# cvg/nice-slam

Hardware: AMD Instinct MI355X
Metric: rendered rays/sec (fwd+bwd) per mapping iter (higher is better)
Workload: dtype f32 (f64 sample placement / depth)

## Files before the change

nice_slam_amd/csrc/nsr_bwd2.h:

```cpp
#pragma once

namespace nsr {

constexpr int kDySlots = 10;
constexpr int kDxMaxWaves = 12;
constexpr int kDxTx = 0, kDxTab = kTile * kTxS, kDxP = kDxTab + 256, kDxDP = kDxP + 48, kDxStg = kDxDP + 48;
static_assert(kDxStg % 4 == 0, "staging regions must stay 16-byte aligned");
constexpr int kDbPart = 288;
NSR_KERNEL void comp_bwd_kernel(const RenderParams P) {
    const int lane = tid() & 63, wave = tid() >> 6, nw = nthreads() >> 6;
    const long long ray = (long long)bid_x() * nw + wave;
    if (ray >= P.n_rays) return;
    const int S = P.S;
    if (!ray_live(P, ray)) {
        if (lane < S) st4(P.draw + (ray * S + lane) * 4, F4{0.f, 0.f, 0.f, 0.f});
        return;
    }
    const bool act = lane < S;
    const long long gp = ray * S + (act ? lane : 0);
    const F4 rw = act ? ld4(P.raw + gp * 4) : F4{0.f, 0.f, 0.f, 0.f};
    const double sc = P.g_scale ? P.g_scale[0] : 1.0;
    const double gD = P.d_depth ? P.d_depth[ray] * sc : 0.0, gV = P.d_var ? P.d_var[ray] * sc : 0.0, dep = P.g_depth[ray];
    float gr = 0.f, gg = 0.f, gb = 0.f;
    if (P.d_rgb) { gr = P.d_rgb[ray * 3 + 0] * (float)sc; gg = P.d_rgb[ray * 3 + 1] * (float)sc; gb = P.d_rgb[ray * 3 + 2] * (float)sc; }
    const double z = act ? P.zvals[gp] : 0.0;
    const Comp cw = comp_weights(rw.w, act, lane);
    const double dz = z - dep;
    float docc = comp_docc(cw, rw, z, dz, gD, gV, gr, gg, gb, act, lane);
    const Pos p = sample_pos(P, ray, z);
    if (!in_bound(P, p.x, p.y, p.z)) docc = 0.f;
    if (act) {
        st4(P.draw + gp * 4, F4{cw.w * gr, cw.w * gg, cw.w * gb, docc});
        store_pos(P, gp, p, z);
    }
}

template <int NTK>
NSR_DEV void gemv_t(f32x4 (&dx)[NTK], const Act<2> &dy, const float *wt, int lane) {
#pragma unroll
    for (int To = 0; To < 2; ++To) {
        f32x4 a[NTK];
#pragma unroll
        for (int Tk = 0; Tk < NTK; ++Tk) a[Tk] = to_v(ld4(wt + ((Tk * 2 + To) * 64 + lane) * 4));
#pragma unroll
        for (int r = 0; r < 4; ++r)
#pragma unroll
            for (int Tk = 0; Tk < NTK; ++Tk) dx[Tk] = mfma16(a[Tk][r], dy.t[To][r], dx[Tk]);
    }
    sched_fence();
}

struct DxIn {
    F4 dr;
    unsigned m0, m1;
};
NSR_DEV DxIn dx_load(const RenderParams &P, const float *acts_pass, long long tile, int pt, int g) {
    DxIn I;
    const long long gp = tile * kTile + pt;
    const long long q = gp < P.n_points_total ? gp : 0;
    I.dr = ld4(P.draw + q * 4);
    const float *mp = acts_pass + ((q >> 4) * kActSlots + kActMask) * 256 + ((q & 15) * 4 + g) * 4;
    I.m0 = __builtin_bit_cast(unsigned, mp[0]);
    I.m1 = __builtin_bit_cast(unsigned, mp[1]);
    return I;
}
NSR_DEV void dx_keep(const DxIn &I) {
    keep_alive(I.dr.w); keep_alive(__builtin_bit_cast(float, I.m1));
}

template <int KIND, bool PARAMS, bool RAYS>
NSR_DEV void dx_pass(const RenderParams &P, int bi, int nbp, int gb) {
    constexpr bool XYZ = KIND != NSR_COARSE;
    constexpr int NOUT = nout_of(KIND);
    char *lds = lds_base();
    const int lane = tid() & 63, wave = uniform(tid() >> 6), nw = nthreads() >> 6;
    const int pt = lane & 15, g = lane >> 4;
    float *aux = reinterpret_cast<float *>(lds);
    float *wt = aux + AUX_FLOATS;
    float *stg = wt + packedT_total(KIND);
    float *Sw = stg + wave * kDxStg;
    const int tail_off = uniform((int)(stg + nw * kDxStg - reinterpret_cast<float *>(lds)));
    const int gl_off = (KIND == NSR_COARSE && P.lds_grid_floats > 0) ? tail_off : -1;
    float *gl = gl_off >= 0 ? reinterpret_cast<float *>(lds) + gl_off : nullptr;
    const bool use_hot = KIND != NSR_COARSE && P.hot_z[KIND] > 0.f && P.grid[KIND].dfeat != nullptr;
    const HotTab hot{use_hot ? tail_off : -1, P.hot_slots};
    int *tcnt = reinterpret_cast<int *>(stg + nw * kDxStg + (KIND == NSR_COARSE ? P.lds_grid_floats : P.hot_slots * kHotRow));
    const GridDev &G = P.grid[KIND];
    const DecDev &D = P.dec[KIND];
    const bool do_grid = G.dfeat != nullptr;
    if (!do_grid && !PARAMS && !RAYS) return;
    const Dbg dbg{P.dbg ? P.dbg + ((long long)gb * kDxMaxWaves + wave) * 64 : nullptr};
    dbg.stamp(0);
    constexpr long long sstride = 256;
    const float *acts_pass = P.acts + (long long)act_pass(KIND) * P.act_tiles * kActSlots * 256;
    const long long ntiles = (P.n_points_total + kTile - 1) / kTile;
    const long long t0 = ntiles * bi / nbp, tend = ntiles * (bi + 1) / nbp;
    long long tile = t0 + wave;
    const bool pre = tile < tend && tile_live(P, tile);
    DxIn cur;
    if (pre) cur = dx_load(P, acts_pass, tile, pt, g);
    copy_f4<AUX_FLOATS / 4>(aux, D.packed);
    copy_f4_dma<packedT_total(KIND) / 4>(wt, D.packed + AUX_FLOATS + packed_total(KIND));
    if (gl) for (int i = tid(); i < P.lds_grid_floats; i += nthreads()) gl[i] = 0.f;
    if (use_hot) hot_init(hot);
    if (tid() == 0) tcnt[0] = nw;
    dma_wait<0>();
    block_sync();
    dbg.stamp(1);
    float *dys = P.dy + (long long)act_pass(KIND) * P.act_tiles * kDySlots * 256;
    const bool need_dc = do_grid || RAYS;
    float aB[kET][3];
#pragma unroll
    for (int k = 0; k < kET; ++k) { aB[k][0] = 0.f; aB[k][1] = 0.f; aB[k][2] = 0.f; }

    auto claim = [&]() -> long long {
        for (;;) {
            int k = 0;
            if (lane == 0) k = atomic_fetch_add_lds_i(tcnt, 1);
            const long long t = t0 + shfl_i(k, 0);
            if (t >= tend || tile_live(P, t)) return t;
        }
    };
    const float dr_scale = (!P.draw_scaled && P.g_scale) ? (float)P.g_scale[0] : 1.f;
    if (!pre) {
        tile = claim();
        if (tile < tend) cur = dx_load(P, acts_pass, tile, pt, g);
    }
    if (tile < tend) dx_keep(cur);
    while (tile < tend) {
        loop_fence();
        const long long nxt = claim();
        const bool has_next = nxt < tend;
        DxIn nx = cur;
        if (has_next) nx = dx_load(P, acts_pass, nxt, pt, g);
        const long long gp = tile * kTile + pt;
        const bool active = gp < P.n_points_total;
        const double *pp = P.pd + (active ? gp : 0) * 4;
        const double cpx = pp[0], cpy = pp[1], cpz = pp[2], cz = pp[3];
        dbg.stamp(2);
        const unsigned mw0 = active ? cur.m0 : 0u, mw1 = active ? cur.m1 : 0u;
        const float dsc = active ? dr_scale : 0.f;
        float d_out[4] = {0.f, 0.f, 0.f, 0.f};
        if (NOUT == 1) d_out[0] = cur.dr.w * dsc;
        else { d_out[0] = cur.dr.x * dsc; d_out[1] = cur.dr.y * dsc; d_out[2] = cur.dr.z * dsc; }
        Act<2> dh;
#pragma unroll
        for (int T = 0; T < 2; ++T) {
            f32x4 v = f4zero();
#pragma unroll
            for (int n = 0; n < (NOUT == 1 ? 1 : 3); ++n) {
                const F4 w = ld4(aux + AUX_WO + n * 32 + 16 * T + 4 * g);
                v[0] = fmaf(w.x, d_out[n], v[0]); v[1] = fmaf(w.y, d_out[n], v[1]);
                v[2] = fmaf(w.z, d_out[n], v[2]); v[3] = fmaf(w.w, d_out[n], v[3]);
            }
            dh.t[T] = v;
        }
        Act<2> dc, dY0, dY3;
        act_zero(dc); act_zero(dY0); act_zero(dY3);
        float *dyp = dys + tile * (kDySlots * 256) + (pt * 4 + g) * 4;
#pragma unroll
        for (int I = 4; I >= 0; --I) {
            if (XYZ && need_dc) gemv_t<2>(dc.t, dh, wt + xyzT_u(I), lane);
            const Act<2> dY = apply_mask(dh, I < 4 ? mw0 : mw1, I < 4 ? 8 * I : 0);
            if (PARAMS && active) {
                st4(dyp + (2 * I) * sstride, to_F4(dY.t[0]));
                st4(dyp + (2 * I + 1) * sstride, to_F4(dY.t[1]));
            }
            if (I == 3) dY3 = dY;
            if (I == 0) dY0 = dY;
            if (!XYZ) {
                if (I == 3 && need_dc) gemv_t<2>(dc.t, dY, wt + nox_mat(NW3C).pk, lane);
                if (I == 0 && need_dc) gemv_t<2>(dc.t, dY, wt + nox_mat(NW0).pk, lane);
            }
            if (I > 0) {
                Act<2> nd;
                act_zero(nd);
                if (XYZ) gemv_t<2>(nd.t, dY, wt + xyzT_wh(I - 1), lane);
                else gemv_t<2>(nd.t, dY, wt + nox_mat(I == 1 ? NW1 : (I == 2 ? NW2 : (I == 3 ? NW3H : NW4))).pk, lane);
                dh = nd;
            }
        }
        dbg.stamp(3);
        const float px = (float)cpx, py = (float)cpy, pz = (float)cpz;
        float dpe[3] = {0.f, 0.f, 0.f};
        if (XYZ && PARAMS && ballot64(active) != 0ull) {
            if (g == 0) { Sw[kDxP + pt] = px; Sw[kDxP + 16 + pt] = py; Sw[kDxP + 32 + pt] = pz; }
            wave_fence();
            const f32x4 qx = to_v(ld4(Sw + kDxP + 4 * g)), qy = to_v(ld4(Sw + kDxP + 16 + 4 * g)), qz = to_v(ld4(Sw + kDxP + 32 + 4 * g));
            f32x4 sx = f4zero(), sy = f4zero(), sz = f4zero();
#pragma unroll
            for (int Tk = 0; Tk < kET; ++Tk) {
                f32x4 e0 = f4zero(), e3 = f4zero();
#pragma unroll
                for (int To = 0; To < 2; ++To) {
                    const f32x4 a0 = to_v(ld4(wt + xyzT_w0() + ((Tk * 2 + To) * 64 + lane) * 4));
                    const f32x4 a3 = to_v(ld4(wt + xyzT_w3e() + ((Tk * 2 + To) * 64 + lane) * 4));
#pragma unroll
                    for (int r = 0; r < 4; ++r) {
                        e0 = mfma16(dY0.t[To][r], a0[r], e0);
                        e3 = mfma16(dY3.t[To][r], a3[r], e3);
                    }
                }
                sched_fence();
                const F4 b = load_b1(aux, 16 * Tk + pt);
                const f32x4 darg = (e0 + e3) * cos_dx4(vfma(qz, splat(b.z), vfma(qy, splat(b.y), qx * splat(b.x))));
#pragma unroll
                for (int r = 0; r < 4; ++r) {
                    aB[Tk][0] = fmaf(darg[r], qx[r], aB[Tk][0]); aB[Tk][1] = fmaf(darg[r], qy[r], aB[Tk][1]);
                    aB[Tk][2] = fmaf(darg[r], qz[r], aB[Tk][2]);
                }
                if (RAYS) { sx = vfma(darg, splat(b.x), sx); sy = vfma(darg, splat(b.y), sy); sz = vfma(darg, splat(b.z), sz); }
            }
            if (RAYS) {
#pragma unroll
                for (int m = 1; m < 16; m <<= 1)
#pragma unroll
                    for (int r = 0; r < 4; ++r) { sx[r] += shfl_xor(sx[r], m); sy[r] += shfl_xor(sy[r], m); sz[r] += shfl_xor(sz[r], m); }
                if (pt == 0) { st4(Sw + kDxDP + 4 * g, to_F4(sx)); st4(Sw + kDxDP + 16 + 4 * g, to_F4(sy)); st4(Sw + kDxDP + 32 + 4 * g, to_F4(sz)); }
                wave_fence();
                dpe[0] = Sw[kDxDP + pt]; dpe[1] = Sw[kDxDP + 16 + pt]; dpe[2] = Sw[kDxDP + 32 + pt];
            }
            wave_fence();
        } else if (XYZ && RAYS) {
            f32x4 dE[kET];
#pragma unroll
            for (int Tk = 0; Tk < kET; ++Tk) dE[Tk] = f4zero();
            gemv_t<kET>(dE, dY0, wt + xyzT_w0(), lane);
            gemv_t<kET>(dE, dY3, wt + xyzT_w3e(), lane);
            float ax = 0.f, ay = 0.f, az = 0.f;
#pragma unroll
            for (int Tk = 0; Tk < kET; ++Tk) {
                const B4 b = load_b4(aux, 4 * Tk + g);
                const f32x4 darg = dE[Tk] * cos_dx4(vfma(splat(pz), b.z, vfma(splat(py), b.y, splat(px) * b.x)));
#pragma unroll
                for (int r = 0; r < 4; ++r) { ax = fmaf(darg[r], b.x[r], ax); ay = fmaf(darg[r], b.y[r], ay); az = fmaf(darg[r], b.z[r], az); }
                sched_fence();
            }
            dpe[0] = red_g(ax); dpe[1] = red_g(ay); dpe[2] = red_g(az);
        }
        dbg.stamp(4);
        Lvl L;
        if (need_dc) L = make_level(G, cpx, cpy, cpz);
        const unsigned live = (do_grid && G.gmask) ? gmask_bits(G, L, g) : 3u;
        float dux = 0.f, duy = 0.f, duz = 0.f;
        if (RAYS) coord_grad(G, L, g, dc, dux, duy, duz);
        dx_keep(nx);
        keep_alive_d(cpx); keep_alive_d(cpy); keep_alive_d(cpz); keep_alive_d(cz);
        dbg.stamp(5);
        if (do_grid)
            scatter_merged(G, L, lane, dc, active, Sw + kDxTx, Sw + kDxTab, gl_off, hot, (float)cz < P.hot_z[KIND], live);
        dbg.stamp(6);
        if (RAYS) {
            double v[6];
            const bool mine = active && g == 0;
            v[0] = mine ? (double)dux * (2.0 * G.inv[0]) + (double)dpe[0] : 0.0;
            v[1] = mine ? (double)duy * (2.0 * G.inv[1]) + (double)dpe[1] : 0.0;
            v[2] = mine ? (double)duz * (2.0 * G.inv[2]) + (double)dpe[2] : 0.0;
            v[3] = v[0] * cz; v[4] = v[1] * cz; v[5] = v[2] * cz;
            if ((P.S & (kTile - 1)) == 0) {
#pragma unroll
                for (int m = 1; m < 16; m <<= 1)
#pragma unroll
                    for (int q = 0; q < 6; ++q) v[q] += shfl_xor_d(v[q], m);
                if (lane == 0 && active) {
                    const long long ray = (long long)((unsigned)gp / (unsigned)P.S);
#pragma unroll
                    for (int q = 0; q < 3; ++q) {
                        atomic_add_global(P.d_rays_o + ray * 3 + q, (float)v[q]);
                        atomic_add_global(P.d_rays_d + ray * 3 + q, (float)v[3 + q]);
                    }
                }
            } else if (mine) {
// ... 305 lines not shown
        const int i = lane & 15, g = lane >> 4;
        if (kWe) {
            img_tile(img, xyz_mat(CD, XW0), 0, WAVE, we[0], i, g); img_tile(img, xyz_mat(CD, XW0), 1, WAVE, we[1], i, g);
            img_tile(img, xyz_mat(CD, XW3E), 0, WAVE, we[2], i, g); img_tile(img, xyz_mat(CD, XW3E), 1, WAVE, we[3], i, g);
        }
        if (kB0) {
#pragma unroll
            for (int T = 0; T < 2; ++T) { const float v = red_g4(vb0[T]); if (g == 0) img[bias_off(KIND, 0) + 16 * T + i] = v; }
        }
        if (WJ) {
            img_tile(img, xyz_mat(CD, hid_of(WJ)), ROW, 0, wh[0], i, g); img_tile(img, xyz_mat(CD, hid_of(WJ)), ROW, 1, wh[1], i, g);
            const float v = red_g4(vb);
            if (g == 0) img[bias_off(KIND, WJ) + 16 * ROW + i] = v;
        }
        if (W2J) {
            img_tile(img, xyz_mat(CD, hid_of(W2J)), ROW, 0, w2[0], i, g); img_tile(img, xyz_mat(CD, hid_of(W2J)), ROW, 1, w2[1], i, g);
            const float v = red_g4(vb2);
            if (g == 0) img[bias_off(KIND, W2J) + 16 * ROW + i] = v;
        }
        if (ROW == 0) {
#pragma unroll
            for (int Tk = 0; Tk < 2; ++Tk)
#pragma unroll
                for (int Tc = 0; Tc < NC; ++Tc) {
                    const f32x4 o = pu[Tk][Tc] + to_v(ld4(comb + (((GJ - 1) * 2 + Tk) * NC + Tc) * 256 + lane * 4));
#pragma unroll
                    for (int r = 0; r < 4; ++r) img[xyz_fcw(CD, GJ - 1) + (16 * Tk + 4 * g + r) * CD + 16 * Tc + i] = o[r];
                }
            if (i == 0) {
#pragma unroll
                for (int Tk = 0; Tk < 2; ++Tk) {
                    if (WJ) {
                        const f32x4 o = pv[Tk] + to_v(ld4(comb + kCombB + (WJ - 1) * 32 + 16 * Tk + 4 * g));
#pragma unroll
                        for (int r = 0; r < 4; ++r) img[xyz_fcb(CD, WJ - 1) + 16 * Tk + 4 * g + r] = o[r];
                    }
                    if (W2J) {
                        const f32x4 o = pv2[Tk] + to_v(ld4(comb + kCombB + (W2J - 1) * 32 + 16 * Tk + 4 * g));
#pragma unroll
                        for (int r = 0; r < 4; ++r) img[xyz_fcb(CD, W2J - 1) + 16 * Tk + 4 * g + r] = o[r];
                    }
                }
            }
        }
        if (kOut) {
            float gsum[NO][NC], bsum[NO];
#pragma unroll
            for (int n = 0; n < NO; ++n) {
#pragma unroll
                for (int T = 0; T < 2; ++T) { const float v = red_g4(wo[n][T]); if (g == 0) img[wo_off(KIND) + n * 32 + 16 * T + i] = v; }
                bsum[n] = red_g4(bo[n]);
                if (lane == 0) img[bo_off(KIND) + n] = bsum[n];
#pragma unroll
                for (int Tc = 0; Tc < NC; ++Tc) gsum[n][Tc] = red_g4(go[n][Tc]);
            }
            if (NOUT == 4 && lane < 32) img[wo_off(KIND) + 3 * 32 + lane] = 0.f;
            if (NOUT == 4 && lane == 0) img[bo_off(KIND) + 3] = 0.f;
#pragma unroll
            for (int kk = 0; kk < 8; ++kk) {
                const int k = 8 * g + kk;
                float wk[NO];
#pragma unroll
                for (int n = 0; n < NO; ++n) wk[n] = params[wo_off(KIND) + n * 32 + k];
#pragma unroll
                for (int Tc = 0; Tc < NC; ++Tc) {
                    float v = 0.f;
#pragma unroll
                    for (int n = 0; n < NO; ++n) v = fmaf(wk[n], gsum[n][Tc], v);
                    img[xyz_fcw(CD, 4) + k * CD + 16 * Tc + i] = v;
                }
                if (i == 0) {
                    float v = 0.f;
#pragma unroll
                    for (int n = 0; n < NO; ++n) v = fmaf(wk[n], bsum[n], v);
                    img[xyz_fcb(CD, 4) + k] = v;
                }
            }
        }
    }
};

template <int WAVE>
struct DwNoxWave {
    static constexpr int LJ = WAVE == NW3C ? 3 : (WAVE == NW3H ? 3 : (WAVE == NW4 ? 4 : WAVE));
    static constexpr bool kMat = WAVE < 6, kBias = kMat && WAVE != NW3H, kOut = WAVE == 6;
    f32x4 w[2][2];
    float vb[2], wo[2], bo, dscale;
    NSR_DEV void init(const RenderParams &P, int) {
        dscale = (!P.draw_scaled && P.g_scale) ? (float)P.g_scale[0] : 1.f;
#pragma unroll
        for (int a = 0; a < 2; ++a) { vb[a] = 0.f; wo[a] = 0.f; w[a][0] = f4zero(); w[a][1] = f4zero(); }
        bo = 0.f;
    }
    struct Ops { f32x4 a[2], x[2]; float dn[4]; };
    NSR_DEV void fetch(const DwSrc s, int lane, Ops &o) {
        const int g = lane >> 4;
        if (kMat) {
            o.a[0] = gop(s.dy + (2 * LJ) * 256, lane); o.a[1] = gop(s.dy + (2 * LJ + 1) * 256, lane);
#pragma unroll
            for (int Tk = 0; Tk < 2; ++Tk)
                o.x[Tk] = gop(s.act + ((WAVE == NW0 || WAVE == NW3C) ? kActC + Tk : 2 * (LJ - 1) + Tk) * 256, lane);
        }
        if (kOut) {
            o.x[0] = gop(s.act + 8 * 256, lane); o.x[1] = gop(s.act + 9 * 256, lane);
#pragma unroll
            for (int q = 0; q < 4; ++q) o.dn[q] = s.dr[(4 * q + g) * 4 + 3] * dscale;
        }
    }
    NSR_DEV void consume(Ops &o, int lane, int nvalid) {
        const int g = lane >> 4;
        if (nvalid < kTile) {
            if (kMat) { rag(o.a[0], g, nvalid); rag(o.a[1], g, nvalid); }
            if (kMat || kOut) { rag(o.x[0], g, nvalid); rag(o.x[1], g, nvalid); }
#pragma unroll
            for (int q = 0; q < 4; ++q) if (kOut && 4 * q + g >= nvalid) o.dn[q] = 0.f;
        }
        if (kMat) {
            if (kBias) { vb[0] += sum4(o.a[0]); vb[1] += sum4(o.a[1]); }
#pragma unroll
            for (int q = 0; q < 4; ++q)
#pragma unroll
                for (int To = 0; To < 2; ++To)
#pragma unroll
                    for (int Tk = 0; Tk < 2; ++Tk) w[To][Tk] = mfma16(o.a[To][q], o.x[Tk][q], w[To][Tk]);
        }
        if (kOut) {
#pragma unroll
            for (int q = 0; q < 4; ++q) { wo[0] = fmaf(o.dn[q], o.x[0][q], wo[0]); wo[1] = fmaf(o.dn[q], o.x[1][q], wo[1]); bo += o.dn[q]; }
        }
    }
    NSR_DEV void flush_products(const float *, float *, int) {}
    NSR_DEV void flush(float *img, const float *, const float *, int lane) {
        const int i = lane & 15, g = lane >> 4;
        if (kMat) {
            const Mat m = nox_mat(WAVE);
#pragma unroll
            for (int To = 0; To < 2; ++To)
#pragma unroll
                for (int Tk = 0; Tk < 2; ++Tk) img_tile(img, m, To, Tk, w[To][Tk], i, g);
            if (kBias) {
#pragma unroll
                for (int T = 0; T < 2; ++T) { const float v = red_g4(vb[T]); if (g == 0) img[nox_b(LJ) + 16 * T + i] = v; }
            }
        }
        if (kOut) {
#pragma unroll
            for (int T = 0; T < 2; ++T) { const float v = red_g4(wo[T]); if (g == 0) img[nox_wo() + 16 * T + i] = v; }
            const float vbo = red_g4(bo);
            if (lane == 0) img[nox_bo()] = vbo;
        }
    }
};

NSR_DEV unsigned long long dw_live_mask(const RenderParams &P, long long bi, long long step, int chunk, long long ntiles, int lane) {
    if (!P.skip_masked) return ~0ull;
    const long long t = bi + ((long long)chunk * 64 + lane) * step;
    bool live = false;
    if (t < ntiles) {
        const unsigned p0 = (unsigned)t * kTile, np = (unsigned)P.n_points_total, pe = p0 + kTile < np ? p0 + kTile : np;
        const unsigned r0 = ray_of_point(P, p0), r1 = ray_of_point(P, pe - 1);
        for (unsigned r = r0; r <= r1; ++r) live = live || P.keep[r] != 0;
    }
    return ballot64(live);
}

template <int KIND, class W>
NSR_DEV void dw_compute(const RenderParams &P, W &Wv, float *ring, int *ctl, float *img, int wave, int lane, int bi, int nbp) {
    typedef DwLay<KIND> Y;
    Wv.init(P, lane & 15);
    const long long ntiles = (P.n_points_total + kTile - 1) / kTile;
    const long long last = ntiles - 1, step = nbp;
    const int ragged = (int)(P.n_points_total & (kTile - 1));
    typename W::Ops ops;
    int k = 0;
    unsigned long long lm = ~0ull;
    const Dbg dbg{P.dbg ? P.dbg + kDwDbgOff + ((long long)bid_x() * kDxMaxWaves + wave) * 64 : nullptr};
    dbg.stamp(0);
    for (long long t = bi; t < ntiles; t += step, ++k) {
        loop_fence();
        dbg.stamp(1);
        if ((k & 63) == 0) lm = dw_live_mask(P, bi, step, k >> 6, ntiles, lane);
        while (flag_load(ctl + (k % kDwLoaders)) <= (k / kDwLoaders)) spin_pause();
        dbg.stamp(2);
        if ((lm >> (k & 63)) & 1ull) {
            Wv.fetch(dw_src<KIND>(ring + (k % kDwRing) * Y::kSlot), lane, ops);
#ifdef NSR_TS
            asm volatile("s_waitcnt lgkmcnt(0)" ::: "memory");
            dbg.stamp(9);
#endif
            Wv.consume(ops, lane, (t == last && ragged) ? ragged : kTile);
        }
        dbg.stamp(3);
        flag_store(ctl + kDwLoaders + wave, k + 1);
        dbg.stamp(4);
    }
    dbg.stamp(5);
    block_sync();
    dbg.stamp(6);
    Wv.flush_products(P.dec[KIND].params, ring, lane);
    block_sync();
    dbg.stamp(7);
    Wv.flush(img, P.dec[KIND].params, ring, lane);
    dbg.stamp(8);
}

template <int KIND>
NSR_DEV void dw_loader(const RenderParams &P, float *ring, int *ctl, int j, int lane, int bi, int nbp) {
    typedef DwLay<KIND> Y;
    const long long ntiles = (P.n_points_total + kTile - 1) / kTile;
    const long long step = nbp;
    int m = 0;
    unsigned long long lm = ~0ull;
    int chunk = -1;
    const Dbg dbg{P.dbg ? P.dbg + kDwDbgOff + ((long long)bid_x() * kDxMaxWaves + kDwCompute + j) * 64 : nullptr};
    dbg.stamp(0);
    for (long long t = bi + j * step; t < ntiles; t += kDwLoaders * step, ++m) {
        loop_fence();
        dbg.stamp(1);
        const int k = kDwLoaders * m + j;
        if ((k >> 6) != chunk) { chunk = k >> 6; lm = dw_live_mask(P, bi, step, chunk, ntiles, lane); }
        if (m >= 1) { dma_wait<0>(); flag_store(ctl + j, m); }
        if (k >= kDwRing) {
            for (;;) {
                int lo = flag_load(ctl + kDwLoaders);
#pragma unroll
                for (int w = 1; w < kDwCompute; ++w) { const int v = flag_load(ctl + kDwLoaders + w); lo = v < lo ? v : lo; }
                if (lo > k - kDwRing) break;
                spin_pause();
            }
        }
        dbg.stamp(2);
        if ((lm >> (k & 63)) & 1ull) {
            dw_issue<KIND>(P, t, ring + (k % kDwRing) * Y::kSlot, lane);
            dbg.stamp(3);
        }
        dbg.stamp(4);
    }
    dma_wait<0>();
    flag_store(ctl + j, m);
    dbg.stamp(5);
    block_sync();
    block_sync();
}

template <int KIND>
NSR_DEV void dw_pass(const RenderParams &P, int bi, int nbp) {
    float *ring = reinterpret_cast<float *>(lds_base());
    int *ctl = reinterpret_cast<int *>(ring + kDwRing * DwLay<KIND>::kSlot);
    const int lane = tid() & 63, wave = uniform(tid() >> 6);
    if (tid() < 16) ctl[tid()] = 0;
    block_sync();
    float *img = P.partials + (long long)bid_x() * P.partial_stride;
#define NSR_DW_CASE(WV)                                                                                         \
    case WV: {                                                                                                  \
        if constexpr (KIND == NSR_COARSE) { DwNoxWave<WV> W; dw_compute<KIND>(P, W, ring, ctl, img, WV, lane, bi, nbp); } \
        else { DwXyzWave<KIND, WV> W; dw_compute<KIND>(P, W, ring, ctl, img, WV, lane, bi, nbp); }                        \
        break;                                                                                                  \
    }
    switch (wave) {
        NSR_DW_CASE(0) NSR_DW_CASE(1) NSR_DW_CASE(2) NSR_DW_CASE(3) NSR_DW_CASE(4) NSR_DW_CASE(5) NSR_DW_CASE(6) NSR_DW_CASE(7)
        default: dw_loader<KIND>(P, ring, ctl, wave - kDwCompute, lane, bi, nbp); break;
    }
#undef NSR_DW_CASE
}

template <int STAGE>
NSR_KERNEL NSR_BOUNDS(64 * kDwWaves) void render_bwd_dw_kernel(const RenderParams P) {
    const int b = bid_x();
    if (STAGE == NSR_STAGE_COARSE) {
        dw_pass<NSR_COARSE>(P, b, nblk_x());
    } else {
        if (b < P.dw_beg[1]) dw_pass<NSR_MIDDLE>(P, b, P.dw_beg[1]);
        else if (b < P.dw_beg[2]) { if (STAGE >= NSR_STAGE_FINE) dw_pass<NSR_FINE>(P, b - P.dw_beg[1], P.dw_beg[2] - P.dw_beg[1]); }
        else { if (STAGE == NSR_STAGE_COLOR) dw_pass<NSR_COLOR>(P, b - P.dw_beg[2], P.dw_beg[3] - P.dw_beg[2]); }
    }
}

struct FinalJob {
    const float *images;
    const float *dbpart;
    float *dparams;
    int kind, nimg, ndx;
};
struct FinalParams {
    FinalJob job[3];
    int stride, overwrite;
};
NSR_DEV void final_store(const FinalParams &R, float *p, float v) { *p = R.overwrite ? v : *p + v; }
NSR_DEV float strided_sum(const float *p, long long stride, int first, int step, int n) {
    float s = 0.f;
    for (int k0 = first; k0 < n; k0 += 16 * step) {
        float v[16];
#pragma unroll
        for (int j = 0; j < 16; ++j) { const int k = k0 + j * step; v[j] = k < n ? p[(long long)k * stride] : 0.f; }
#pragma unroll
        for (int j = 0; j < 16; ++j) if (k0 + j * step < n) s += v[j];
    }
    return s;
}

NSR_KERNEL void bwd_finalize_kernel(const FinalParams R) {
    const FinalJob J = R.job[bid_y()];
    float *red = reinterpret_cast<float *>(lds_base());
    const int kind = J.kind, cd = cdim_of(kind);
    const int total = param_total(kind);
    const int t = tid(), nt = nthreads();
    const int lane = t & 63, slice = t >> 6, nslice = nt >> 6;
    const int e = bid_x() * 64 + lane;
    if (bid_x() * 64 >= total) return;
    float s = 0.f;
    if (e < total) {
        const int rb = kind != NSR_COARSE ? e - xyz_B(cd) : -1;
        if (rb >= 0 && rb < 3 * kE) {
            const int d = rb / kE, ch = rb - d * kE;
            s = strided_sum(J.dbpart + d * 96 + ch, kDbPart, slice, nslice, J.ndx);
        } else {
            s = strided_sum(J.images + e, R.stride, slice, nslice, J.nimg);
        }
    }
    red[t] = s;
    block_sync();
    if (slice == 0 && e < total) {
        for (int k = 1; k < nslice; ++k) s += red[k * 64 + lane];
        final_store(R, J.dparams + e, s);
    }
}

}
```

nice_slam_amd/csrc/nsr_fwd2.h:

```cpp
#pragma once

namespace nsr {

NSR_KERNEL void fwd_sample_kernel(const RenderParams P) {
    double *zs = reinterpret_cast<double *>(lds_base());
    const int lane = tid() & 63, wave = tid() >> 6, nw = nthreads() >> 6;
    const long long ray = (long long)bid_x() * nw + wave;
    const int S = P.S;
    double *zw = zs + wave * 64;
    if (ray >= P.n_rays) return;
    const bool act = lane < S;
    const int k = act ? lane : 0;
    const bool guided = depth_guided(P);
    double z = sample_candidate(P, ray, k, guided);
    if (P.n_surface > 0 && guided) {
        if (act) zw[lane] = z;
        wave_fence();
        const int rank = stable_rank(zw, S, k, z);
        wave_fence();
        if (act) zw[rank] = z;
        wave_fence();
        z = act ? zw[lane] : 0.0;
    }
    if (!act) return;
    const long long gq = ray * S + lane;
    P.zvals[gq] = z;
    store_pos(P, gq, sample_pos(P, ray, z), z);
}

template <int KIND, bool SAVE>
NSR_DEV void fwd_pass(const RenderParams &P, int bi, int nbp) {
    float *aux = reinterpret_cast<float *>(lds_base());
    float *wl = aux + AUX_FLOATS;
    int *cnt = reinterpret_cast<int *>(wl + packed_total(KIND));
    const int lane0 = tid() & 63, wave = tid() >> 6;
    const DecDev &D = P.dec[KIND];
    const Dbg dbg{P.dbg ? P.dbg + ((long long)bid_x() * 12 + wave) * 64 : nullptr};
    dbg.stamp(0);
    load_aux<KIND>(aux, D.packed);
    copy_f4_dma<packed_total(KIND) / 4>(wl, D.packed + AUX_FLOATS);
    if (tid() == 0) cnt[0] = 0;
    dma_wait<0>();
    block_sync();
    dbg.stamp(1);
    const long long ntiles = (P.n_points_total + kTile - 1) / kTile;
    const long long t0 = ntiles * bi / nbp, t1 = ntiles * (bi + 1) / nbp;
    for (;;) {
        int take = 0;
        if (lane0 == 0) take = atomic_fetch_add_lds_i(cnt, 1);
        const long long tile = t0 + shfl_i(take, 0);
        if (tile >= t1) break;
        if (!tile_live(P, tile)) continue;
        loop_fence();
        const int lane = opaque_i(lane0), pt = lane & 15, g = lane >> 4;
        const long long gp = tile * kTile + pt;
        const bool active = gp < P.n_points_total;
        const double *pp = P.pd + (active ? gp : 0) * 4;
        const double px = pp[0], py = pp[1], pz = pp[2];
        dbg.stamp(2);
        const long long sp = (SAVE && active) ? gp : -1;
        float *scr = P.draw + gp * 4;
        if (KIND == NSR_COARSE) {
            const Lvl L = make_level(P.grid[NSR_COARSE], px, py, pz);
            const Act<2> c = gather_feat(P.grid[NSR_COARSE], L, g);
            float o[1];
            const ActSink sk = act_sink(P, 0, sp, g);
            mlp_nox_fwd<SAVE>(wl, aux, c, lane, o, &sk);
            if (active && g == 0) scr[0] = o[0];
        } else {
            const float fx = (float)px, fy = (float)py, fz = (float)pz;
            if (KIND == NSR_MIDDLE) {
                const Lvl Lm = make_level(P.grid[NSR_MIDDLE], px, py, pz);
                const Act<2> cm = gather_feat(P.grid[NSR_MIDDLE], Lm, g);
                float om[1];
                const ActSink sk = act_sink(P, 0, sp, g);
                mlp_xyz_fwd<NSR_MIDDLE, SAVE>(wl, aux, fx, fy, fz, cm, lane, om, &sk);
                if (active && g == 0) scr[0] = om[0];
            } else if (KIND == NSR_FINE) {
                const Lvl Lf = make_level(P.grid[NSR_FINE], px, py, pz);
                const Act<2> cf = gather_feat(P.grid[NSR_FINE], Lf, g);
                const Lvl Lm = make_level(P.grid[NSR_MIDDLE], px, py, pz);
                const Act<2> cm = gather_feat(P.grid[NSR_MIDDLE], Lm, g);
                Act<4> cc;
                cc.t[0] = cf.t[0]; cc.t[1] = cf.t[1]; cc.t[2] = cm.t[0]; cc.t[3] = cm.t[1];
                float of[1];
                const ActSink sk = act_sink(P, 1, sp, g);
                mlp_xyz_fwd<NSR_FINE, SAVE>(wl, aux, fx, fy, fz, cc, lane, of, &sk);
                if (active && g == 0) scr[1] = of[0];
            } else {
                const Lvl Lc = make_level(P.grid[NSR_COLOR], px, py, pz);
                const Act<2> ccol = gather_feat(P.grid[NSR_COLOR], Lc, g);
                float oc[4];
                const ActSink sk = act_sink(P, 2, sp, g);
                mlp_xyz_fwd<NSR_COLOR, SAVE>(wl, aux, fx, fy, fz, ccol, lane, oc, &sk);
                if (active && g == 0) { float *rw = P.raw + gp * 4; rw[0] = oc[0]; rw[1] = oc[1]; rw[2] = oc[2]; }
            }
        }
        dbg.stamp(3);
    }
    dbg.stamp(9);
}

template <int STAGE, bool SAVE>
NSR_KERNEL NSR_BOUNDS(768) void render_fwd_pass_kernel(const RenderParams P) {
    const int b = bid_x();
    if (STAGE == NSR_STAGE_COARSE) {
        fwd_pass<NSR_COARSE, SAVE>(P, b, nblk_x());
    } else {
        if (b < P.pass_beg[1]) fwd_pass<NSR_MIDDLE, SAVE>(P, b, P.pass_beg[1]);
        else if (b < P.pass_beg[2]) { if (STAGE >= NSR_STAGE_FINE) fwd_pass<NSR_FINE, SAVE>(P, b - P.pass_beg[1], P.pass_beg[2] - P.pass_beg[1]); }
        else { if (STAGE == NSR_STAGE_COLOR) fwd_pass<NSR_COLOR, SAVE>(P, b - P.pass_beg[2], P.pass_beg[3] - P.pass_beg[2]); }
    }
}

template <int STAGE>
NSR_KERNEL void fwd_composite_kernel(const RenderParams P) {
    double *red = reinterpret_cast<double *>(lds_base());
    const int lane = tid() & 63, wave = tid() >> 6, nw = nthreads() >> 6;
    const long long rayq = (long long)bid_x() * nw + wave;
    const int S = P.S;
    double lterm = 0.0;
    if (rayq < P.n_rays && !ray_live(P, rayq)) {
        if (lane == 0) {
            P.depth[rayq] = 0.0; P.var[rayq] = 0.0;
            P.rgb[rayq * 3 + 0] = 0.f; P.rgb[rayq * 3 + 1] = 0.f; P.rgb[rayq * 3 + 2] = 0.f;
            if (P.loss && P.dl_depth) P.dl_depth[rayq] = 0.0;
            if (P.loss && P.dl_rgb) { P.dl_rgb[rayq * 3 + 0] = 0.f; P.dl_rgb[rayq * 3 + 1] = 0.f; P.dl_rgb[rayq * 3 + 2] = 0.f; }
        }
        if (P.loss && P.dl_depth && lane < S) st4(P.draw + (rayq * S + lane) * 4, F4{0.f, 0.f, 0.f, 0.f});
    } else if (rayq < P.n_rays) {
        const bool act = lane < S;
        const long long gq = rayq * S + (act ? lane : 0);
        const bool kp = !P.loss || !P.keep || P.keep[rayq];
        const float gd = (P.loss && P.loss_depth) ? P.loss_depth[rayq] : 0.f;
        float gtc[3] = {0.f, 0.f, 0.f};
        if (P.loss && STAGE == NSR_STAGE_COLOR && P.gt_color) { gtc[0] = P.gt_color[rayq * 3 + 0]; gtc[1] = P.gt_color[rayq * 3 + 1]; gtc[2] = P.gt_color[rayq * 3 + 2]; }
        double qx = 0.0, qy = 0.0, qz = 0.0, zq = 0.0;
        F4 rw = F4{0.f, 0.f, 0.f, 0.f};
        bool ins = true;
        if (act) {
            const double *pq = P.pd + gq * 4;
            qx = pq[0]; qy = pq[1]; qz = pq[2]; zq = pq[3];
            const float *scr = P.draw + gq * 4;
            float occ = scr[0];
            if (STAGE >= NSR_STAGE_FINE) occ = scr[1] + scr[0];
            if (STAGE == NSR_STAGE_COLOR) { const float *rc = P.raw + gq * 4; rw.x = rc[0]; rw.y = rc[1]; rw.z = rc[2]; }
            ins = in_bound(P, qx, qy, qz);
            rw.w = ins ? occ : 100.f;
            st4(P.raw + gq * 4, rw);
        }
        const Comp c = comp_weights(rw.w, act, lane);
        const RayOut o = composite(c, rw, zq);
        if (lane == 0) {
            P.depth[rayq] = o.depth;
            P.var[rayq] = o.var;
            P.rgb[rayq * 3 + 0] = o.cr; P.rgb[rayq * 3 + 1] = o.cg; P.rgb[rayq * 3 + 2] = o.cb;
        }
        if (P.loss) {
            const RayLoss L = mapping_loss_ray<STAGE>(P, kp, gd, gtc, o.depth, o.cr, o.cg, o.cb);
            lterm = L.term;
            if (lane == 0) {
                if (P.dl_depth) P.dl_depth[rayq] = L.gD;
                if (P.dl_rgb) { P.dl_rgb[rayq * 3 + 0] = L.g3[0]; P.dl_rgb[rayq * 3 + 1] = L.g3[1]; P.dl_rgb[rayq * 3 + 2] = L.g3[2]; }
            }
            if (P.dl_depth) {
                float docc = comp_docc(c, rw, zq, o.dz, L.gD, 0.0, L.g3[0], L.g3[1], L.g3[2], act, lane);
                if (!ins) docc = 0.f;
                if (act) st4(P.draw + gq * 4, F4{c.w * L.g3[0], c.w * L.g3[1], c.w * L.g3[2], docc});
            }
        }
    }
    if (P.loss) {
        if (lane == 0) red[wave] = lterm;
        block_sync();
        if (tid() == 0) {
            double s = 0.0;
            for (int w = 0; w < nw; ++w) s += red[w];
            if (s != 0.0) atomic_add_global_d(P.loss, s);
        }
    }
}

}
```

nice_slam_amd/csrc/nsr_kernels.h:

```cpp
#pragma once
#include "nsr_dev.h"
#include "nsr_layout.h"
#include "../../include/nsr.h"

namespace nsr {

template <int NT>
struct Act { f32x4 t[NT]; };

NSR_DEV f32x4 f4zero() { f32x4 v = {0.f, 0.f, 0.f, 0.f}; return v; }
NSR_DEV f32x4 to_v(F4 a) { f32x4 v = {a.x, a.y, a.z, a.w}; return v; }
NSR_DEV F4 to_F4(f32x4 v) { return F4{v[0], v[1], v[2], v[3]}; }
template <int NT> NSR_DEV void act_zero(Act<NT> &a) {
#pragma unroll
    for (int T = 0; T < NT; ++T) a.t[T] = f4zero();
}

NSR_DEV double tmax(double a, double b) { return (a > b || a != a) ? a : b; }
NSR_DEV double tmin(double a, double b) { return (a < b || a != a) ? a : b; }

struct GridDev {
    const float *feat;
    float *dfeat;
    const unsigned char *gmask;
    int Z, Y, X;
    double lo[3];
    double ext[3];
    double inv[3];
};

struct DecDev {
    const float *params;
    const float *packed;
    float *dparams;
};

struct RenderParams {
    int stage, n_samples, n_surface, S;
    long long n_rays;
    int rays_per_block, tiles_per_block;
    long long n_groups;
    const float *rays_o, *rays_d, *gt_depth, *gt_max;
    double blo[3], bhi[3];
    float t_uniform[NSR_MAX_SAMPLES];
    double t_surface[NSR_MAX_SAMPLES];
    GridDev grid[4];
    DecDev dec[4];
    double *depth, *var;
    float *rgb, *raw;
    double *zvals;
    float *acts;
    int acts_masks_only;
    long long n_points_total;
    long long act_tiles;
    const double *d_depth, *d_var, *g_depth;
    const double *g_scale;
    const float *d_rgb;
    float *d_rays_o, *d_rays_d;
    float *partials;
    int partial_stride;
    const float *loss_depth;
    const float *gt_color;
    const unsigned char *keep;
    double *loss;
    double *dl_depth;
    float *dl_rgb;
    float w_color;
    long long *dbg;
    float *dy;
    float *draw;
    double *pd;
    float *pf;
    float *dbpart;
    int dw_beg[4];
    int dx_beg[4];
    int draw_scaled;
    int skip_masked;
    int lds_grid_floats;
    float hot_z[4];
    int hot_slots;
    unsigned s_magic;
    int pass_beg[4];
    const double *points;
    long long n_points;
    float *out_points;
};

NSR_DEV bool ray_live(const RenderParams &P, long long ray) { return !P.skip_masked || uniform_load_u8(P.keep + ray) != 0u; }
NSR_DEV unsigned ray_of_point(const RenderParams &P, unsigned x) {
    return P.s_magic ? (unsigned)(((unsigned long long)x * P.s_magic) >> 32) : x;
}
NSR_DEV bool tile_live(const RenderParams &P, long long tile) {
    if (!P.skip_masked) return true;
    const unsigned p0 = (unsigned)uniform((int)tile) * kTile, np = (unsigned)P.n_points_total, pe = p0 + kTile < np ? p0 + kTile : np;
    const unsigned r0 = ray_of_point(P, p0), r1 = ray_of_point(P, pe - 1);
    bool live = false;
    for (unsigned r = r0; r <= r1; ++r) live = live || uniform_load_u8(P.keep + r) != 0u;
    return live;
}

template <int KIND>
NSR_DEV float aux_value(const float *__restrict__ flat, int idx) {
    float v = 0.f;
    if (idx < AUX_V) {
        const int i = idx >> 5, o = idx & 31;
        v = flat[bias_off(KIND, i) + o];
    } else if (idx < AUX_WO) {
        if (is_xyz(KIND)) { const int i = (idx - AUX_V) >> 5, o = idx & 31; v = flat[fcb_off(KIND, i) + o]; }
    } else if (idx < AUX_BO) {
        const int n = (idx - AUX_WO) >> 5, k = idx & 31;
        if (n < nout_of(KIND)) v = flat[wo_off(KIND) + n * 32 + k];
    } else if (idx < AUX_BM) {
        const int n = idx - AUX_BO;
        if (n < nout_of(KIND)) v = flat[bo_off(KIND) + n];
    } else if (is_xyz(KIND)) {
        const int rel = idx - AUX_BM, ch = (rel >> 4) * 4 + (rel & 3), d = (rel >> 2) & 3;
        if (ch < kE && d < 3) v = flat[B_off(KIND) + d * kE + ch];
    }
    return v;
}

template <int KIND>
NSR_KERNEL void pack_kernel(const float *__restrict__ flat, float *__restrict__ packed) {
    const int gidx = bid_x() * nthreads() + tid();
    if (gidx >= packed_buf_total(KIND)) return;
    if (gidx < AUX_FLOATS) { packed[gidx] = aux_value<KIND>(flat, gidx); return; }
    const int idx = gidx - AUX_FLOATS;
    float v = 0.f;
    if (idx < packed_total(KIND)) {
#pragma unroll
        for (int id = 0; id < nmat_of(KIND); ++id) {
            const Mat m = mat_of(KIND, id);
            const int rel = idx - m.pk;
            if (rel >= 0 && rel < m.nt * 512) {
                const int r = rel & 3, lane = (rel >> 2) & 63, Tp = (rel >> 8) & 1, T = rel >> 9;
                const int o = 16 * Tp + (lane & 15);
                const int k = 16 * T + 4 * (lane >> 4) + r;
                if (k < m.kcols) v = flat[m.off + o * m.stride + m.kbeg + k];
            }
        }
    } else {
        const int idt = idx - packed_total(KIND);
#pragma unroll
        for (int id = 0; id < nmatT_of(KIND); ++id) {
            const Mat m = matT_of(KIND, id);
            const int rel = idt - m.pk;
            if (rel >= 0 && rel < m.nt * 512) {
                const int r = rel & 3, lane = (rel >> 2) & 63, To = (rel >> 8) & 1, Tk = rel >> 9;
                const int o = 16 * To + 4 * (lane >> 4) + r;
                const int k = 16 * Tk + (lane & 15);
                if (k < m.kcols) v = flat[m.off + o * m.stride + m.kbeg + k];
            }
        }
    }
    packed[gidx] = v;
}

template <int NF4, int B = 4>
NSR_DEV void copy_f4(float *dst, const float *__restrict__ src) {
    const int nt = nthreads();
    int t = tid();
    for (; t + (B - 1) * nt < NF4; t += B * nt) {
        F4 v[B];
#pragma unroll
        for (int k = 0; k < B; ++k) v[k] = ld4(src + 4 * (t + k * nt));
#pragma unroll
        for (int k = 0; k < B; ++k) st4(dst + 4 * (t + k * nt), v[k]);
    }
    for (; t < NF4; t += nt) st4(dst + 4 * t, ld4(src + 4 * t));
}
template <int NF4>
NSR_DEV void copy_f4_dma(float *dst, const float *__restrict__ src) {
    static_assert(NF4 % 64 == 0, "whole 1 KB pieces");
    const int nt = nthreads(), lane = tid() & 63;
    for (int t = tid(); t < NF4; t += nt) dma16(src + 4 * t, dst + 4 * (t - lane), lane);
}
template <int KIND>
NSR_DEV void load_aux(float *aux, const float *__restrict__ packed) { copy_f4<AUX_FLOATS / 4>(aux, packed); }

NSR_DEV double ray_far_bb(const RenderParams &P, long long ray) {
    double far = 0.0;
#pragma unroll
    for (int a = 0; a < 3; ++a) {
        const double o = (double)P.rays_o[ray * 3 + a], d = (double)P.rays_d[ray * 3 + a];
        const double t0 = (P.blo[a] - o) / d, t1 = (P.bhi[a] - o) / d;
        const double m = tmax(t0, t1);
        far = (a == 0) ? m : tmin(far, m);
    }
    return far + 0.01;
}

NSR_DEV bool depth_guided(const RenderParams &P) { return (P.gt_depth != nullptr) && (P.stage != NSR_STAGE_COARSE); }

NSR_DEV double sample_candidate(const RenderParams &P, long long ray, int k, bool guided) {
    const double far_bb = ray_far_bb(P, ray);
    if (!guided) {
        const float tk = P.t_uniform[k];
        const float near_part = 0.01f * (1.f - tk);
        return (double)near_part + far_bb * (double)tk;
    }
    const float g = P.gt_depth[ray];
    const float gmax = P.gt_max[0];
    if (k < P.n_samples) {
        const float tk = P.t_uniform[k];
        const double cap = (double)(gmax * 1.2f);
        const double far = tmin(tmax(far_bb, 0.0), cap);
        const float near = g * 0.01f;
        return (double)(near * (1.f - tk)) + far * (double)tk;
    }
    const double s = P.t_surface[k - P.n_samples];
    if (g > 0.f) {
        const double e0 = (double)(0.95f * g), e1 = (double)(1.05f * g);
        return e0 * (1.0 - s) + e1 * s;
    }
    return 0.001 * (1.0 - s) + (double)gmax * s;
}

NSR_DEV int stable_rank(const double *zr, int S, int k, double v) {
    int rank = 0;
#pragma unroll 16
    for (int j = 0; j < S; ++j) {
        const double u = zr[j];
        rank += (u < v || (u == v && j < k)) ? 1 : 0;
    }
    return rank;
}

struct Pos { double x, y, z; };
NSR_DEV Pos sample_pos(const RenderParams &P, long long ray, double z) {
    Pos p;
    p.x = (double)P.rays_o[ray * 3 + 0] + (double)P.rays_d[ray * 3 + 0] * z;
    p.y = (double)P.rays_o[ray * 3 + 1] + (double)P.rays_d[ray * 3 + 1] * z;
    p.z = (double)P.rays_o[ray * 3 + 2] + (double)P.rays_d[ray * 3 + 2] * z;
    return p;
}
NSR_DEV bool in_bound(const RenderParams &P, double x, double y, double z) {
    return (x > P.blo[0]) && (x < P.bhi[0]) && (y > P.blo[1]) && (y < P.bhi[1]) && (z > P.blo[2]) && (z < P.bhi[2]);
}
NSR_DEV void store_pos(const RenderParams &P, long long gq, const Pos &p, double z) {
    double *q = P.pd + gq * 4;
    q[0] = p.x; q[1] = p.y; q[2] = p.z; q[3] = z;
    st4(P.pf + gq * 4, F4{(float)p.x, (float)p.y, (float)p.z, 0.f});
}

NSR_DEV void compute_z(const RenderParams &P, long long ray0, double *ztmp, double *zbuf) {
    const int S = P.S, npts = P.rays_per_block * S;
    const bool guided = depth_guided(P);
    for (int t = tid(); t < npts; t += nthreads()) {
        const int r = t / S, k = t - r * S;
        const long long ray = ray0 + r;
        ztmp[t] = ray < P.n_rays ? sample_candidate(P, ray, k, guided) : 0.0;
// ... 1832 lines not shown
```

Before: 4.771 million.

## Balance tile ranges across blocks by counting live tiles under ray masking

Blocks now split only the live (unmasked) tiles evenly, instead of taking equal contiguous slices of all tiles. A wave-level scan over the keep mask counts and locates the live tiles, and the forward, dx and dw passes all use the resulting range. dw switches from a strided tile assignment to contiguous ranges, and the live-mask check becomes cheaper when each tile spans few rays. This aims to fix load imbalance when many rays are masked, at the cost of an extra scan over the mask in every block.

```diff
diff --git a/nice_slam_amd/csrc/nsr_bwd2.h b/nice_slam_amd/csrc/nsr_bwd2.h
--- a/nice_slam_amd/csrc/nsr_bwd2.h
+++ b/nice_slam_amd/csrc/nsr_bwd2.h
@@ -93,17 +93,17 @@
     dbg.stamp(0);
     constexpr long long sstride = 256;
     const float *acts_pass = P.acts + (long long)act_pass(KIND) * P.act_tiles * kActSlots * 256;
-    const long long ntiles = (P.n_points_total + kTile - 1) / kTile;
-    const long long t0 = ntiles * bi / nbp, tend = ntiles * (bi + 1) / nbp;
+    copy_f4_dma<packedT_total(KIND) / 4>(wt, D.packed + AUX_FLOATS + packed_total(KIND));
+    copy_f4<AUX_FLOATS / 4>(aux, D.packed);
+    int t0, tend;
+    live_range(P, bi, nbp, t0, tend);
     long long tile = t0 + wave;
     const bool pre = tile < tend && tile_live(P, tile);
     DxIn cur;
     if (pre) cur = dx_load(P, acts_pass, tile, pt, g);
-    copy_f4<AUX_FLOATS / 4>(aux, D.packed);
-    copy_f4_dma<packedT_total(KIND) / 4>(wt, D.packed + AUX_FLOATS + packed_total(KIND));
     if (gl) for (int i = tid(); i < P.lds_grid_floats; i += nthreads()) gl[i] = 0.f;
     if (use_hot) hot_init(hot);
-    if (tid() == 0) tcnt[0] = nw;
+    if (tid() == 0) tcnt[0] = t0 + nw;
     dma_wait<0>();
     block_sync();
     dbg.stamp(1);
@@ -117,7 +117,7 @@
         for (;;) {
             int k = 0;
             if (lane == 0) k = atomic_fetch_add_lds_i(tcnt, 1);
-            const long long t = t0 + shfl_i(k, 0);
+            const long long t = shfl_i(k, 0);
             if (t >= tend || tile_live(P, t)) return t;
         }
     };
@@ -729,34 +729,24 @@
     }
 };
 
-NSR_DEV unsigned long long dw_live_mask(const RenderParams &P, long long bi, long long step, int chunk, long long ntiles, int lane) {
-    if (!P.skip_masked) return ~0ull;
-    const long long t = bi + ((long long)chunk * 64 + lane) * step;
-    bool live = false;
-    if (t < ntiles) {
-        const unsigned p0 = (unsigned)t * kTile, np = (unsigned)P.n_points_total, pe = p0 + kTile < np ? p0 + kTile : np;
-        const unsigned r0 = ray_of_point(P, p0), r1 = ray_of_point(P, pe - 1);
-        for (unsigned r = r0; r <= r1; ++r) live = live || P.keep[r] != 0;
-    }
-    return ballot64(live);
-}
-
 template <int KIND, class W>
 NSR_DEV void dw_compute(const RenderParams &P, W &Wv, float *ring, int *ctl, float *img, int wave, int lane, int bi, int nbp) {
     typedef DwLay<KIND> Y;
     Wv.init(P, lane & 15);
     const long long ntiles = (P.n_points_total + kTile - 1) / kTile;
-    const long long last = ntiles - 1, step = nbp;
+    const long long last = ntiles - 1;
+    int t0, t1;
+    live_range(P, bi, nbp, t0, t1);
     const int ragged = (int)(P.n_points_total & (kTile - 1));
     typename W::Ops ops;
     int k = 0;
     unsigned long long lm = ~0ull;
     const Dbg dbg{P.dbg ? P.dbg + kDwDbgOff + ((long long)bid_x() * kDxMaxWaves + wave) * 64 : nullptr};
     dbg.stamp(0);
-    for (long long t = bi; t < ntiles; t += step, ++k) {
+    for (long long t = t0; t < t1; ++t, ++k) {
         loop_fence();
         dbg.stamp(1);
-        if ((k & 63) == 0) lm = dw_live_mask(P, bi, step, k >> 6, ntiles, lane);
+        if ((k & 63) == 0) lm = live_mask64(P, t, ntiles, lane);
         while (flag_load(ctl + (k % kDwLoaders)) <= (k / kDwLoaders)) spin_pause();
         dbg.stamp(2);
         if ((lm >> (k & 63)) & 1ull) {
@@ -785,17 +775,18 @@
 NSR_DEV void dw_loader(const RenderParams &P, float *ring, int *ctl, int j, int lane, int bi, int nbp) {
     typedef DwLay<KIND> Y;
     const long long ntiles = (P.n_points_total + kTile - 1) / kTile;
-    const long long step = nbp;
+    int t0, t1;
+    live_range(P, bi, nbp, t0, t1);
     int m = 0;
     unsigned long long lm = ~0ull;
     int chunk = -1;
     const Dbg dbg{P.dbg ? P.dbg + kDwDbgOff + ((long long)bid_x() * kDxMaxWaves + kDwCompute + j) * 64 : nullptr};
     dbg.stamp(0);
-    for (long long t = bi + j * step; t < ntiles; t += kDwLoaders * step, ++m) {
+    for (long long t = t0 + j; t < t1; t += kDwLoaders, ++m) {
         loop_fence();
         dbg.stamp(1);
         const int k = kDwLoaders * m + j;
-        if ((k >> 6) != chunk) { chunk = k >> 6; lm = dw_live_mask(P, bi, step, chunk, ntiles, lane); }
+        if ((k >> 6) != chunk) { chunk = k >> 6; lm = live_mask64(P, t0 + 64LL * chunk, ntiles, lane); }
         if (m >= 1) { dma_wait<0>(); flag_store(ctl + j, m); }
         if (k >= kDwRing) {
             for (;;) {
diff --git a/nice_slam_amd/csrc/nsr_fwd2.h b/nice_slam_amd/csrc/nsr_fwd2.h
--- a/nice_slam_amd/csrc/nsr_fwd2.h
+++ b/nice_slam_amd/csrc/nsr_fwd2.h
@@ -39,16 +39,16 @@
     dbg.stamp(0);
     load_aux<KIND>(aux, D.packed);
     copy_f4_dma<packed_total(KIND) / 4>(wl, D.packed + AUX_FLOATS);
-    if (tid() == 0) cnt[0] = 0;
+    int t0, t1;
+    live_range(P, bi, nbp, t0, t1);
+    if (tid() == 0) cnt[0] = t0;
     dma_wait<0>();
     block_sync();
     dbg.stamp(1);
-    const long long ntiles = (P.n_points_total + kTile - 1) / kTile;
-    const long long t0 = ntiles * bi / nbp, t1 = ntiles * (bi + 1) / nbp;
     for (;;) {
         int take = 0;
         if (lane0 == 0) take = atomic_fetch_add_lds_i(cnt, 1);
-        const long long tile = t0 + shfl_i(take, 0);
+        const long long tile = shfl_i(take, 0);
         if (tile >= t1) break;
         if (!tile_live(P, tile)) continue;
         loop_fence();
diff --git a/nice_slam_amd/csrc/nsr_kernels.h b/nice_slam_amd/csrc/nsr_kernels.h
--- a/nice_slam_amd/csrc/nsr_kernels.h
+++ b/nice_slam_amd/csrc/nsr_kernels.h
@@ -90,13 +90,104 @@
 NSR_DEV unsigned ray_of_point(const RenderParams &P, unsigned x) {
     return P.s_magic ? (unsigned)(((unsigned long long)x * P.s_magic) >> 32) : x;
 }
+NSR_DEV void tile_rays(const RenderParams &P, unsigned tile, unsigned &r0, unsigned &r1) {
+    const unsigned p0 = tile * kTile, np = (unsigned)P.n_points_total, pe = p0 + kTile < np ? p0 + kTile : np;
+    r0 = ray_of_point(P, p0); r1 = ray_of_point(P, pe - 1);
+}
 NSR_DEV bool tile_live(const RenderParams &P, long long tile) {
     if (!P.skip_masked) return true;
-    const unsigned p0 = (unsigned)uniform((int)tile) * kTile, np = (unsigned)P.n_points_total, pe = p0 + kTile < np ? p0 + kTile : np;
-    const unsigned r0 = ray_of_point(P, p0), r1 = ray_of_point(P, pe - 1);
+    unsigned r0, r1;
+    tile_rays(P, (unsigned)uniform((int)tile), r0, r1);
     bool live = false;
     for (unsigned r = r0; r <= r1; ++r) live = live || uniform_load_u8(P.keep + r) != 0u;
     return live;
+}
+template <bool FEW>
+NSR_DEV bool tile_live_lane(const RenderParams &P, long long t, long long ntiles) {
+    const bool in = t < ntiles;
+    unsigned r0, r1;
+    tile_rays(P, in ? (unsigned)t : 0u, r0, r1);
+    bool live = (P.keep[r0] | P.keep[r1]) != 0;
+    if (!FEW) for (unsigned r = r0 + 1; r < r1; ++r) live = live || P.keep[r] != 0;
+    return in && live;
+}
+NSR_DEV unsigned long long live_mask64(const RenderParams &P, long long first, long long ntiles, int lane) {
+    if (!P.skip_masked) return ~0ull;
+    return ballot64(P.S >= kTile ? tile_live_lane<true>(P, first + lane, ntiles) : tile_live_lane<false>(P, first + lane, ntiles));
+}
+
+constexpr int kLrChunks = 8;
+constexpr long long kLrMaxItems = 64LL * 64 * kLrChunks;
+template <int MODE>
+NSR_DEV bool item_live(const RenderParams &P, long long i, long long n) {
+    if (MODE == 0) { const bool in = i < n; return in && P.keep[in ? i : 0] != 0; }
+    return tile_live_lane<MODE == 1>(P, i, n);
+}
+struct LiveStep { bool lv[kLrChunks]; };
+template <int MODE>
+NSR_DEV LiveStep live_step(const RenderParams &P, long long first, long long n, int lane) {
+    LiveStep s;
+#pragma unroll
+    for (int j = 0; j < kLrChunks; ++j) s.lv[j] = item_live<MODE>(P, first + 64 * j + lane, n);
+    return s;
+}
+NSR_DEV int live_count(const LiveStep &s) {
+    int n = 0;
+#pragma unroll
+    for (int j = 0; j < kLrChunks; ++j) n += __builtin_popcountll(ballot64(s.lv[j]));
+    return n;
+}
+NSR_DEV int live_pick(const LiveStep &s, int first, int k, int lane) {
+    int t = first;
+    bool found = false;
+#pragma unroll
+    for (int j = 0; j < kLrChunks; ++j) {
+        const unsigned long long m = ballot64(s.lv[j]);
+        const int n = __builtin_popcountll(m);
+        if (!found && k < n) {
+            const bool me = s.lv[j] && __builtin_popcountll(m & ((1ull << lane) - 1ull)) == k;
+            t = first + 64 * j + __builtin_ctzll(ballot64(me));
+            found = true;
+        }
+        if (!found) k -= n;
+    }
+    return t;
+}
+template <int MODE>
+NSR_DEV void live_range_items(const RenderParams &P, int bi, int nbp, long long n, int m, int &t0, int &t1) {
+    const int lane = tid() & 63;
+    constexpr long long kStep = 64LL * kLrChunks;
+    int Li = 0, before = 0;
+    int nstep = 0;
+    for (long long c = 0; c < n; c += kStep, ++nstep) {
+        if (lane == nstep) before = Li;
+        Li += live_count(live_step<MODE>(P, c, n, lane));
+    }
+    if (Li == (int)n) return;
+    const long long L = (long long)Li * m;
+    const int a = (int)(L * bi / nbp), b = (int)(L * (bi + 1) / nbp);
+    int tb[2] = {(int)(n * m), (int)(n * m)};
+#pragma unroll 1
+    for (int e = 0; e < 2; ++e) {
+        const int want = e ? b : a;
+        if (want >= L) continue;
+        const int wi = want / m;
+        const unsigned long long le = ballot64(lane < nstep && before <= wi);
+        const int st = 63 - __builtin_clzll(le);
+        const int first = st * (int)kStep;
+        tb[e] = live_pick(live_step<MODE>(P, first, n, lane), first, wi - shfl_i(before, st), lane) * m + (want - wi * m);
+    }
+    t0 = uniform(tb[0]); t1 = uniform(tb[1]);
+}
+NSR_DEV void live_range(const RenderParams &P, int bi, int nbp, int &t0, int &t1) {
+    const long long T = (P.n_points_total + kTile - 1) / kTile;
+    t0 = (int)(T * bi / nbp); t1 = (int)(T * (bi + 1) / nbp);
+    if (!P.skip_masked) return;
+    if (P.S % kTile == 0) { if (P.n_rays <= kLrMaxItems) live_range_items<0>(P, bi, nbp, P.n_rays, P.S / kTile, t0, t1); }
+    else if (T <= kLrMaxItems) {
+        if (P.S >= kTile) live_range_items<1>(P, bi, nbp, T, 1, t0, t1);
+        else live_range_items<2>(P, bi, nbp, T, 1, t0, t1);
+    }
 }
 
 template <int KIND>
```

Result: slower. 4.372 million (-8.4%).
